# nilsfriess/dune-ddm

Measured on AMD Instinct MI355X. Metric: preconditioned CG iterations/sec (two-level additive Schwarz), 3D Poisson 10M DoF, higher is better.
Workload: dtype f64

## Files before the change

### dune-ddm_amd/__init__.py

```python
from __future__ import annotations

import ctypes
import os

import numpy as np

_HERE = os.path.dirname(os.path.abspath(__file__))
LIB_PATH = os.path.join(_HERE, "libddm_hip.so")

GENEO_AVAILABLE = True

DDM_OK, DDM_EINVAL, DDM_EHIP, DDM_ENOTIMPL, DDM_ENUMERIC, DDM_ECOMM = 0, -1, -2, -3, -4, -5
MULTI_ENGINES = ("levels", "xcd", "xcd1")


class DdmError(RuntimeError):
    def __init__(self, code, msg):
        super().__init__(f"ddm_hip error {code}: {msg}")
        self.code = code


class SolveResult(ctypes.Structure):
    _fields_ = [("iterations", ctypes.c_int32), ("converged", ctypes.c_int32), ("def0", ctypes.c_double),
                ("reduction", ctypes.c_double), ("elapsed_s", ctypes.c_double)]
# ... 43 lines not shown
    "ddm_galerkin_set_inverse": (_I32, [_P, _P, _P]),
    "ddm_csr_destroy": (None, [_P]),
    "ddm_csr_rows": (_I64, [_P]),
    "ddm_csr_nnz": (_I64, [_P]),
    "ddm_csr_mv": (_I32, [_P, _P, _P, _P]),
    "ddm_csr_usmv": (_I32, [_P, _P, _D, _P, _P]),
    "ddm_csr_mm": (_I32, [_P, _P, _I32, _P, _P]),
    "ddm_csr_row_order_tiled_host": (_I32, [_I64, _P, _P, _P, _P]),
    "ddm_dia_build_and_apply_host": (_I32, [_I64, _P, _P, _P, _P, _P, _I64, _P, _P]),
    "ddm_dia_windows_host": (_I32, [_I64, _P, _P, _P, _I64, _P, _I64, _P, _P]),
    "ddm_dia_codes_host": (_I32, [_I64, _P, _P, _P, _I32, _I64, _P, _P, _P, _P]),
    "ddm_ilu0_solve_multi": (_I32, [_P, _P, _I32, _P, _P]),
    "ddm_ilu0_solve_multi_f32": (_I32, [_P, _P, _I32, _P, _P]),
    "ddm_ilu0_create": (_I32, [_P, _P, _I64, _P, _PP]),
    "ddm_ilu0_destroy": (None, [_P]),
    "ddm_ilu0_solve": (_I32, [_P, _P, _P, _P]),
    "ddm_ilu0_debug_stamps": (_I32, [_P, _P, _P, _P, _P]),
    "ddm_ilu0_status": (_I32, [_P, _P, ctypes.POINTER(ctypes.c_int)]),
    "ddm_ilu0_peek_status": (_I32, [_P]),
    "ddm_ilu0_set_status": (_I32, [_P, _I32]),
    "ddm_halo_exchange_to": (_I32, [_P, _P, _P, _P]),
    "ddm_schwarz_local_solver": (_P, [_P]),
    "ddm_ilu0_pipe_trace": (_I32, [_P, _P, _P, _P, _P, _P, _I64, ctypes.POINTER(ctypes.c_int64)]),
    "ddm_ilu0_num_levels": (_I64, [_P, _I32]),
    "ddm_ilu0_wait": (_I32, [_P, _P]),
    "ddm_ilu0_box_check": (_I32, [_P, _P]),
    "ddm_ilu0_box_info": (_I32, [_P, _P, ctypes.c_int64, _P]),
    "ddm_ilu0_solve_tail": (_I32, [_P, _P, _P, _P, _P, _P]),
    "ddm_ilu0_engine": (_I32, [_P]),
    "ddm_chol_create": (_I32, [_P, _P, _I64, _P, _D, _PP]),
    "ddm_ilu0_is_direct": (_I32, [_P]),
    "ddm_ilu0_refinement": (_I32, [_P, _P]),
    "ddm_ilu0_sn_pivots": (_I32, [_P, _P, _P]),
    "ddm_sn_host_create": (_I32, [_I64, _P, _P, _I64, _P, _PP]),
    "ddm_sn_host_destroy": (None, [_P]),
    "ddm_sn_host_sizes": (_I32, [_P, _I64, _P, ctypes.POINTER(ctypes.c_double)]),
    "ddm_sn_host_get": (_I32, [_P, _I64, _P, _P, _P, _P, _P, _P]),
    "ddm_ilu0_nnz": (_I64, [_P]),
    "ddm_chol_host_create": (_I32, [_I64, _P, _P, _P, _I64, _P, _PP]),
    "ddm_direct_host_create": (_I32, [_I64, _P, _P, _P, _I64, _P, _I32, _PP]),
    "ddm_direct_create": (_I32, [_P, _P, _I64, _P, _I32, _D, _PP]),
    "ddm_chol_host_destroy": (None, [_P]),
    "ddm_chol_host_nnz": (_I64, [_P]),
    "ddm_chol_host_nnz_factor": (_I64, [_P]),
    "ddm_chol_host_flops": (_D, [_P]),
    "ddm_chol_host_get": (_I32, [_P, _P, _P, _P, _P]),
# ... 457 lines not shown
        return {"blocks": [tuple(int(v) for v in out[3 + 5 * b:8 + 5 * b]) for b in range(int(out[0]))], "grid": int(out[1]),
                "nested": SchwarzPreconditioner.ENGINES[int(out[2])] if out[2] >= 0 else None}

    def solve_tail(self, d, x, scale=None, add=None):
        self.ctx.check(self.ctx.lib.ddm_ilu0_solve_tail(self.ctx.h, self.h, _ptr(d), _ptr(x), _ptr(scale) if scale is not None else None,
                                                       _ptr(add) if add is not None else None))

    def wait(self):
        self.ctx.check(self.ctx.lib.ddm_ilu0_wait(self.ctx.h, self.h))

    def debug_stamps(self, d, x):
        out = np.zeros(8, dtype=np.uint64)
        self.ctx.check(self.ctx.lib.ddm_ilu0_debug_stamps(self.ctx.h, self.h, _ptr(d), _ptr(x), _hp(out)))
        return out

    def pipe_trace(self, d, x):
        nt = ctypes.c_int64()
        self.ctx.check(self.ctx.lib.ddm_ilu0_pipe_trace(self.ctx.h, self.h, None, None, None, None, 0, ctypes.byref(nt)))
        out = np.zeros((nt.value, 272), dtype=np.uint64)
        meta = np.zeros((nt.value, 2), dtype=np.int32)
        self.ctx.check(self.ctx.lib.ddm_ilu0_pipe_trace(self.ctx.h, self.h, _ptr(d), _ptr(x), _hp(out), _hp(meta), nt.value, ctypes.byref(nt)))
        return out, meta

    def engine(self):
        return SchwarzPreconditioner.ENGINES[int(self.ctx.lib.ddm_ilu0_engine(self.h))]

    def status(self):
        st = ctypes.c_int()
        self.ctx.check(self.ctx.lib.ddm_ilu0_status(self.ctx.h, self.h, ctypes.byref(st)))
        return st.value

    def factors(self):
        out = np.empty(self.nnz, dtype=np.float64)
        self.ctx.check(self.ctx.lib.ddm_ilu0_get_factors_host(self.ctx.h, self.h, _hp(out)))
        return out

    def __del__(self):
        try:
            if self.h and self.ctx.h:
                self.ctx.lib.ddm_ilu0_destroy(self.h)
        except Exception:
            pass


class Halo:
    COPY, ADD = 0, 1
# ... 756 lines not shown
```

### dune-ddm_amd/csrc/engine_pipe.hpp

```cpp

static int build_pipe_schedule(ddm_ctx *ctx, ddm_ilu0 *F)
{
  const ddm_csr *A = F->A;
  DDMCHECK(ilu0_sync_host_factor(ctx, F));
  pipe::Options opt;
  if (const char *e = std::getenv("DDM_PIPE_DELTA")) opt.delta = std::atoi(e);
  if (const char *e = std::getenv("DDM_PIPE_SPAN")) opt.max_span = std::atoi(e);
  if (const char *e = std::getenv("DDM_PIPE_REUSE")) opt.vote = std::atoi(e);
  int spread_env = -1;
  if (const char *e = std::getenv("DDM_PIPE_SPREAD")) spread_env = std::atoi(e);
  pipe::Schedule S;
  const int nb = (int)F->h_block_ptr.size() - 1;
  if (!pipe::build(A->nrows, A->h_rp.data(), A->h_ci.data(), F->h_lu.data(), F->h_diag.data(), nb, F->h_block_ptr.data(), opt, S)) {
    if (std::getenv("DDM_PIPE_VERBOSE")) std::fprintf(stderr, "[ddm] pipe engine not applicable: %s\n", S.error.c_str());
    return DDM_OK;
  }
  auto E = std::make_unique<PipeEngine>();
  E->ngroups = nb;
  E->stats = S.stats;
  E->spread = spread_env >= 0 ? spread_env : (nb < 8 && S.stats.max_rows_per_level > 48.0 * 64.0 ? 1 : 0);
  E->nposU = S.nposU;
  DDMCHECK(upload(ctx, S.groups.data(), (int64_t)S.groups.size(), E->groups));
  DDMCHECK(upload(ctx, S.tasks.data(), (int64_t)S.tasks.size(), E->tasks));
  DDMCHECK(upload(ctx, S.stream.data(), (int64_t)S.stream.size(), E->stream));
  DDMCHECK(upload(ctx, S.koff.data(), (int64_t)S.koff.size(), E->koff));
  DDMCHECK(upload(ctx, S.posU.data(), (int64_t)S.posU.size(), E->posU));
  {
    std::vector<int64_t> slot(S.slot[0]);
    slot.insert(slot.end(), S.slot[1].begin(), S.slot[1].end());
    DDMCHECK(upload(ctx, slot.data(), (int64_t)slot.size(), E->slot));
  }
  {
    std::vector<int32_t> rowU((size_t)std::max<int64_t>(S.nposU, 1), -1);
    for (size_t i = 0; i < S.posU.size(); ++i) rowU[(size_t)S.posU[i]] = (int32_t)i;
    DDMCHECK(upload(ctx, rowU.data(), (int64_t)rowU.size(), E->rowU));
  }
  HIPCHECK(ctx, E->ypos.alloc(S.nposL));
  HIPCHECK(ctx, E->xpos.alloc(S.nposU));
  HIPCHECK(ctx, dev_memset(E->ypos, 0, sizeof(double) * (size_t)std::max<int64_t>(S.nposL, 1)));
  HIPCHECK(ctx, dev_memset(E->xpos, 0, sizeof(double) * (size_t)std::max<int64_t>(S.nposU, 1)));
  const size_t pbytes = sizeof(unsigned long long) * 16 * std::max<size_t>(S.tasks.size(), 1);
  HIPCHECK(ctx, E->progress.alloc((int64_t)(pbytes / sizeof(unsigned long long))));
  HIPCHECK(ctx, dev_memset(E->progress, 0, pbytes));
  HIPCHECK(ctx, E->queue.alloc(32 * 4 * (int64_t)nb));
  HIPCHECK(ctx, dev_memset(E->queue, 0, sizeof(unsigned) * 32 * 4 * (size_t)nb));
  DDMCHECK(ilu0_alloc_xstate(ctx, F));
  HIPCHECK(ctx, hipFuncSetAttribute((const void *)k_trsv_pipe<false>, hipFuncAttributeMaxDynamicSharedMemorySize, (int)PIPE_LDS_BYTES));
  HIPCHECK(ctx, hipFuncSetAttribute((const void *)k_trsv_pipe<true>, hipFuncAttributeMaxDynamicSharedMemorySize, (int)PIPE_LDS_BYTES));
  int per_cu = 0;
  HIPCHECK(ctx, hipOccupancyMaxActiveBlocksPerMultiprocessor(&per_cu, (const void *)k_trsv_pipe<false>, 64 * PIPE_WAVES, PIPE_LDS_BYTES));
  per_cu = std::max(1, std::min(per_cu, 2));
  if (const char *e = std::getenv("DDM_PIPE_WG_PER_CU")) per_cu = std::max(1, std::min(per_cu, std::atoi(e)));
  E->grid = per_cu * (ctx->num_cu / 8 * 8);
  if (std::getenv("DDM_PIPE_VERBOSE")) {
    const pipe::Stats &st = S.stats;
    std::fprintf(stderr,
                 "[ddm] pipe schedule: %lld rows, tasks %lld+%lld, steps %lld+%lld (lane occupancy %.3f / %.3f), entries %lld: local %.3f self-global %.3f remote %.3f, "
                 "stream %.1f MB (%.2fx of 12 B/entry), max producers %lld, max steps %lld, regrouped %lld, levels <= %lld, rows/level <= %.0f, spread %d, grid %d\n",
                 (long long)st.rows, (long long)st.ntasks[0], (long long)st.ntasks[1], (long long)st.nsteps[0], (long long)st.nsteps[1],
                 (double)st.rows / (64.0 * std::max<int64_t>(st.nsteps[0], 1)), (double)st.rows / (64.0 * std::max<int64_t>(st.nsteps[1], 1)), (long long)st.entries,
                 (double)st.entries_local / std::max<int64_t>(st.entries, 1), (double)st.entries_self_global / std::max<int64_t>(st.entries, 1),
                 (double)st.entries_remote / std::max<int64_t>(st.entries, 1), S.stream.size() / 1e6, S.stream.size() / (12.0 * std::max<int64_t>(st.entries, 1)),
                 (long long)st.max_prod, (long long)st.max_steps, (long long)st.regrouped, (long long)st.max_levels, st.max_rows_per_level, E->spread, E->grid);
  }
  F->pipe = std::move(E);
  return DDM_OK;
}

static unsigned perm_grid(ddm_ctx *ctx, int64_t npos) { return (unsigned)std::max<int64_t>(1, std::min<int64_t>((npos + PERM_TILE - 1) / PERM_TILE, (int64_t)ctx->num_cu * 16)); }
static hipError_t enqueue_pipe(ddm_ctx *ctx, ddm_ilu0 *F, const double *d, double *x, unsigned *err, unsigned long long *stamps, const double *scale = nullptr,
                               const double *add = nullptr, hipEvent_t add_ready = nullptr)
{
  const PipeEngine &E = *F->pipe;
  PipeParams P;
  P.ngroups = E.ngroups;
  P.groups = E.groups;
  P.tasks = E.tasks;
  P.stream = E.stream;
  P.koff = E.koff;
  P.d = d;
  P.ypos = E.ypos;
  P.xpos = E.xpos;
  P.progress = E.progress;
  P.queue = E.queue;
  P.st = F->xstate;
  P.err = err;
// ... 11 lines not shown
```

### dune-ddm_amd/csrc/local_factor.hpp

```cpp

struct TriSchedule {
  int64_t nlev = 0;
  std::vector<LevelDesc> desc;
  dbuf<int32_t> rows;
  dbuf<int32_t> cols;
  dbuf<double> vals;
  dbuf<double> dinv;
  dbuf<float> vals_f32, dinv_f32;
  dbuf<LevelDesc> d_desc;
  struct Launch {
    int first, count;
    bool small;
  };
  std::vector<Launch> plan;
  int64_t ell_entries = 0;
  dbuf<int32_t> blk_off, blk_nlev;
  std::vector<int32_t> h_blk_nlev;
};

struct TriCsr {
  int64_t nlev = 0;
  std::vector<CsrLevel> desc;
  int64_t nrows = 0, entries = 0;
  dbuf<int32_t> rows;
// ... 33 lines not shown
  dbuf<GroupDesc> groups;
  dbuf<LevelDesc> desc;
  dbuf<int64_t> flag_off;
  dbuf<int32_t> rows, cols;
  dbuf<double> vals, dinv;
  dbuf<unsigned> flags;
  dbuf<double> dperm;
  dbuf<int64_t> lpos;
};

struct PipeEngine {
  int ngroups = 0;
  dbuf<pipe::Group> groups;
  dbuf<pipe::Task> tasks;
  dbuf<unsigned char> stream;
  dbuf<int32_t> koff, posU, rowU;
  dbuf<double> ypos, xpos;
  dbuf<unsigned long long> progress;
  dbuf<unsigned> queue;
  dbuf<int64_t> slot;
  int64_t nposU = 0;
  int spread = 0;
  int grid = 0;
  pipe::Stats stats;
};

struct BoxEngine {
  int nblocks = 0;
  int64_t nshell = 0, nprod = 0;
  dbuf<box::Block> blocks;
  dbuf<box::StepTab> steps;
  dbuf<double> stream;
  dbuf<unsigned long long> einfo;
  dbuf<double> E, ext_val;
  dbuf<int32_t> ext_col;
  dbuf<double> xs;
  dbuf<unsigned long long> prog;
  dbuf<unsigned> queue;
  unsigned long long *dbg = nullptr;
  int64_t n = 0, stream_len = 0, xs_len = 0, prog_len = 0, einfo_len = 0;
  dbuf<int64_t> srp;
  dbuf<int32_t> sci, srow;
  dbuf<double> sva, ds, xsol;
  ddm_csr *shell_csr = nullptr;
  ddm_ilu0 *shell = nullptr;
  int grid = 0;
// ... 147 lines not shown
```

### dune-ddm_amd/csrc/local_solve.hpp

```cpp

static int ilu0_prepare_engine(ddm_ctx *ctx, ddm_ilu0 *F)
{
  DDMCHECK(ilu0_join(ctx, F));
  if (F->engine == Engine::Box && F->box->shell) return ilu0_prepare_engine(ctx, F->box->shell);
  if (F->engine == Engine::Xcd2 && !F->xcd) return build_xcd_schedule(ctx, F);
  return DDM_OK;
}

static void enqueue_sn_panel(ddm_ctx *ctx, const ddm_ilu0 *F, int w, const double *D, int64_t ldd, double *X, int64_t ldx, double *work, double *yvec, unsigned *err)
{
  const SnDirect &S = *F->sn;
  const int64_t n = F->n;
  const dim3 grid(grid_for(n * w));
  hipLaunchKernelGGL(k_perm_gather, grid, dim3(WG), 0, ctx->stream, n, w, S.f->d_perm, D, ldd, work);
  sn::solve(*S.f, ctx->stream, w, work, w, yvec, err);
  hipLaunchKernelGGL(k_perm_scatter, grid, dim3(WG), 0, ctx->stream, n, w, S.f->d_perm, (const double *)work, X, ldx);
  for (int it = 0; it < S.refine_steps; ++it) {
    hipLaunchKernelGGL(k_residual_rowmajor, dim3((unsigned)((n * (int64_t)w + WG - 1) / WG)), dim3(WG), 0, ctx->stream, n, w, (const int64_t *)S.ref_rp, (const int32_t *)S.ref_ci,
                       (const double *)S.ref_va, (const double *)X, ldx, D, ldd, S.pr, (int64_t)w);
    hipLaunchKernelGGL(k_perm_gather, grid, dim3(WG), 0, ctx->stream, n, w, S.f->d_perm, (const double *)S.pr, (int64_t)w, work);
    sn::solve(*S.f, ctx->stream, w, work, w, yvec, err);
    hipLaunchKernelGGL(k_perm_scatter_add, grid, dim3(WG), 0, ctx->stream, n, w, S.f->d_perm, (const double *)work, X, ldx);
  }
}
// ... 74 lines not shown
  DDMCHECK(ilu0_join(ctx, F));
  if (!F->pipe) DDMCHECK(build_pipe_schedule(ctx, F));
  if (!F->pipe) return fail(ctx, DDM_EINVAL, "pipe engine not applicable to this matrix");
  const int64_t nt = F->pipe->stats.ntasks[0] + F->pipe->stats.ntasks[1];
  *ntasks = nt;
  if (!out_host) return DDM_OK;
  if (capacity_tasks < nt || !d || !x || d == x) return fail(ctx, DDM_EINVAL, "ddm_ilu0_pipe_trace: bad arguments");
  dbuf<unsigned long long> st;
  HIPCHECK(ctx, st.alloc(PIPE_STAMP_WORDS * (nt + 1)));
  HIPCHECK(ctx, hipMemsetAsync(st, 0, sizeof(unsigned long long) * PIPE_STAMP_WORDS * (size_t)(nt + 1), ctx->stream));
  (void)enqueue_pipe(ctx, F, d, x, F->err, st);
  int rc = ddm_memcpy_d2h(ctx, out_host, st, (int64_t)sizeof(unsigned long long) * PIPE_STAMP_WORDS * nt);
  if (!rc && meta_host) {
    std::vector<pipe::Task> tasks((size_t)nt);
    rc = ddm_memcpy_d2h(ctx, tasks.data(), F->pipe->tasks, (int64_t)sizeof(pipe::Task) * nt);
    for (int64_t t = 0; t < nt && !rc; ++t) {
      meta_host[2 * t] = tasks[(size_t)t].group;
      meta_host[2 * t + 1] = tasks[(size_t)t].sweep;
    }
  }
  return rc;
}

static int ilu0_is_pipe(ddm_ctx *ctx, ddm_ilu0 *F, bool *yes)
{
  *yes = false;
  if (!F || F->n == 0) return DDM_OK;
  DDMCHECK(ilu0_prepare_engine(ctx, F));
  *yes = F->engine == Engine::Pipe;
  return DDM_OK;
}

static int sn_check_valid(ddm_ctx *ctx, const ddm_ilu0 *F)
{
  if (F->sn && F->sn->invalid) return fail(ctx, DDM_ENUMERIC, "sparse direct solver (device): the factor is invalid after a failed refresh");
  return DDM_OK;
}

static int ilu0_solve_epilogue(ddm_ctx *ctx, ddm_ilu0 *F, const double *d, double *x, const double *scale, const double *add, hipEvent_t add_ready = nullptr)
{
  if (F && F->n == 0) return DDM_OK;
  if (!F || !d || !x || d == x) return fail(ctx, DDM_EINVAL, "ddm_ilu0_solve: bad arguments (d and x must not alias)");
  DDMCHECK(sn_check_valid(ctx, F));
  if (add_ready) {
    bool pipe_engine = false;
    DDMCHECK(ilu0_is_pipe(ctx, F, &pipe_engine));
// ... 97 lines not shown
```

### dune-ddm_amd/csrc/trsv_pipe_host.hpp

```cpp
#pragma once
#include "host_vec.hpp"
#include <algorithm>
#include <cstdint>
#include <cstring>
#include <functional>
#include <queue>
#include <string>
#include <thread>
#include <vector>

#if defined(__HIPCC__)
#define PIPE_HD __host__ __device__
#else
#define PIPE_HD
#endif

namespace pipe {

constexpr int LANES = 64;
constexpr int RING = 16;
constexpr int RING_Z = RING * LANES * 8;
constexpr int RING_BYTES = RING_Z + LANES * 8;
constexpr int ZERO_POS = RING_Z / 8;
constexpr int FIRST_POS = ZERO_POS + LANES;
constexpr int MIN_W = 14;
inline int32_t ring_op(int step, int lane) { return (int32_t)(((step % RING) * LANES + lane) * 8); }
constexpr int32_t PAD_OP = RING_Z;
constexpr int MAXPROD = 112;
constexpr int HDR_REQ0 = 8;
constexpr int MAX_W = 26;

struct Task {
  int64_t tile_off;
  int64_t pos_base;
  int64_t koff_base;
  int32_t nsteps, nprod, group, sweep;
  int32_t W, first_kib, pad0;
  int32_t start_level, pad[2];
  int32_t prod[MAXPROD];
};
static_assert(sizeof(Task) == 512, "Task layout");
struct Group {
  int32_t task0[2], ntask[2];
};

struct Geometry {
  int W = 0, idx_pieces = 0, val_pieces = 0, tile_bytes = 0;
  constexpr Geometry() = default;
  PIPE_HD constexpr explicit Geometry(int w_) : W(w_ > MIN_W ? w_ : MIN_W), idx_pieces((W + 3) / 4), val_pieces((W + 1) / 2), tile_bytes(1024 * (1 + idx_pieces + val_pieces)) {}
  static constexpr int FIXED_VAL = MIN_W / 2, FIXED_IDX = (MIN_W + 3) / 4, FIXED_KIB = 1 + FIXED_VAL + FIXED_IDX;
  PIPE_HD int val_piece(int q2) const { return q2 < FIXED_VAL ? 1 + q2 : FIXED_KIB + (q2 - FIXED_VAL); }
  PIPE_HD int idx_piece(int q4) const { return q4 < FIXED_IDX ? 1 + FIXED_VAL + q4 : FIXED_KIB + (val_pieces - FIXED_VAL) + (q4 - FIXED_IDX); }
  PIPE_HD int val_off(int u, int lane) const { return 1024 * val_piece(u >> 1) + lane * 16 + (u & 1) * 8; }
  PIPE_HD int idx_off(int u, int lane) const { return 1024 * idx_piece(u >> 2) + lane * 16 + (u & 3) * 4; }
};

PIPE_HD inline int64_t row_slot(int64_t tile_kib, int W, int lane) { return tile_kib << 16 | (int64_t)W << 8 | lane; }

struct Options {
  int delta = 24;
  int vote = 1;
  int pack_steps = 64;
  int max_span = 256;
};

struct Stats {
  int64_t ntasks[2] = {0, 0}, nsteps[2] = {0, 0};
  int64_t rows = 0, entries = 0, entries_local = 0, entries_self_global = 0, entries_remote = 0;
  int64_t max_prod = 0, max_steps = 0, regrouped = 0, nchains[2] = {0, 0};
  int64_t max_levels = 0;
  double max_rows_per_level = 0.0;
};

struct Schedule {
  Geometry geo;
  std::vector<Group> groups;
  std::vector<Task> tasks;
  hvec<unsigned char> stream;
  std::vector<int32_t> koff;
  std::vector<int32_t> rowL;
  std::vector<int32_t> posU;
  std::vector<int64_t> slot[2];
  int64_t nposL = 0, nposU = 0;
  Stats stats;
  std::string error;
};

namespace detail {

struct BlockSweep {
  struct TaskRec {
    int32_t start0 = 0, nsteps = 0, W = 1;
    std::vector<int32_t> stepW;
    std::vector<int32_t> rows;
    std::vector<int32_t> prod;
  };
  std::vector<TaskRec> tasks;
  std::vector<int32_t> task_of, step_of, lane_of;
  int64_t nchains = 0;
  bool cyclic = false, too_many_prod = false;
  int dissolve_rounds = 0;
  int32_t nlev = 0;
};

template <class Deps>
static void build_block_sweep(int64_t nb, bool upper, const Deps &deps, const Options &opt, BlockSweep &B)
{
  std::vector<int32_t> lev(nb, 0), chain(nb, -1), coff(nb, 0), ndep(nb, 0);
  std::vector<uint8_t> claimed(nb, 0), nochain(nb, 0);
  struct Chain {
    int32_t head, start, len;
  };
  std::vector<Chain> chains;
  std::vector<int64_t> cptr, pptr;
  std::vector<int32_t> crow(nb), pidx, freerows, comp;
  std::vector<uint8_t> is_free;
  int64_t nc = 0;
  int32_t ncomp = 0;
  auto sweep_key = [&](int32_t row) { return upper ? (int32_t)(nb - 1 - row) : row; };
  for (;;) {
    chains.clear();
    chains.reserve(nb / 16 + 16);
// ... 204 lines not shown
      return sweep_key(chains[a].head) < sweep_key(chains[b].head);
    });
    int32_t smin = 0x7fffffff, emax = 0;
    for (int64_t m = mptr[k]; m < mptr[k + 1]; ++m) {
      smin = std::min(smin, chains[members[m]].start);
      emax = std::max(emax, chains[members[m]].start + chains[members[m]].len);
    }
    bool fits = !protos.empty();
    if (fits) {
      const Proto &P = protos.back();
      if (std::max(P.end, emax) - std::min(P.start0, smin) > opt.max_span && !P.chains.empty()) fits = false;
      if (fits && opt.vote == 0 && (int)P.chains.size() + (int)(mptr[k + 1] - mptr[k]) > LANES) fits = false;
      if (fits) fits = place(mptr[k], mptr[k + 1], false);
    }
    if (!fits) new_task();
    place(mptr[k], mptr[k + 1], true);
    for (int64_t s = sptr[k]; s < sptr[k + 1]; ++s)
      if (--indeg[sidx[s]] == 0) ready.push(ckey[sidx[s]]);
  }
  if (emitted != ncomp) {
    B.cyclic = true;
    return;
  }
  const int64_t per_pack = (int64_t)opt.pack_steps * LANES;
  const int64_t npack = ((int64_t)freerows.size() + per_pack - 1) / per_pack;
  const int64_t ntask = npack + (int64_t)protos.size();
  B.task_of.assign(nb, -1);
  B.step_of.assign(nb, -1);
  B.lane_of.assign(nb, -1);
  for (int64_t f = 0; f < (int64_t)freerows.size(); ++f) {
    const int32_t i = freerows[f];
    B.task_of[i] = (int32_t)(f / per_pack);
    B.step_of[i] = (int32_t)((f % per_pack) / LANES);
    B.lane_of[i] = (int32_t)(f % LANES);
  }
  for (int64_t p = 0; p < (int64_t)protos.size(); ++p)
    for (size_t a = 0; a < protos[p].chains.size(); ++a) {
      const int32_t c = protos[p].chains[a];
      for (int32_t k = 0; k < chains[c].len; ++k) {
        const int32_t i = crow[cptr[c] + k];
        B.task_of[i] = (int32_t)(npack + p);
        B.step_of[i] = chains[c].start + k - protos[p].start0;
        B.lane_of[i] = protos[p].lanes[a];
      }
    }
  B.tasks.resize(ntask);
  for (int64_t t = 0; t < ntask; ++t) {
    auto &T = B.tasks[t];
    if (t < npack) {
      const int64_t cnt = std::min<int64_t>(per_pack, (int64_t)freerows.size() - t * per_pack);
      T.start0 = 0;
      T.nsteps = (int32_t)((cnt + LANES - 1) / LANES);
    } else {
      T.start0 = protos[t - npack].start0;
      T.nsteps = protos[t - npack].end - protos[t - npack].start0;
    }
    T.rows.assign((size_t)T.nsteps * LANES, -1);
    T.stepW.assign((size_t)T.nsteps, 1);
  }
  for (int64_t i = 0; i < nb; ++i) {
    const int32_t t = B.task_of[i];
    B.tasks[t].rows[(size_t)B.step_of[i] * LANES + B.lane_of[i]] = (int32_t)i;
    B.tasks[t].W = std::max(B.tasks[t].W, ndep[i]);
    B.tasks[t].stepW[B.step_of[i]] = std::max(B.tasks[t].stepW[B.step_of[i]], ndep[i]);
    deps(i, [&](int64_t j) {
      const int32_t tj = B.task_of[j];
      if (tj > t) B.cyclic = true;
      if (tj != t) B.tasks[t].prod.push_back(tj);
    });
  }
  for (auto &T : B.tasks) {
    std::sort(T.prod.begin(), T.prod.end());
    T.prod.erase(std::unique(T.prod.begin(), T.prod.end()), T.prod.end());
    if ((int)T.prod.size() > MAXPROD) B.too_many_prod = true;
  }
}

}

inline bool build(int64_t n, const int64_t *rp, const int32_t *ci, const double *lu, const int64_t *diag, int nblocks,
                  const int64_t *block_ptr, Options opt, Schedule &S, int nthreads = 0)
{
  using detail::BlockSweep;
  S = Schedule();
  int W = 1;
  for (int64_t i = 0; i < n; ++i) W = std::max<int>(W, (int)std::max(diag[i] - rp[i], rp[i + 1] - diag[i] - 1));
  if (W > MAX_W) {
    S.error = "triangular rows wider than the tile format";
    return false;
  }
// ... 26 lines not shown
      detail::build_block_sweep(nb, upper, deps, opt, B);
      Options o2 = opt;
      while (B.too_many_prod && !B.cyclic && o2.max_span > 24) {
        o2.max_span /= 2;
        B = BlockSweep();
        detail::build_block_sweep(nb, upper, deps, o2, B);
        regrouped[(size_t)b * 2 + sweep] += 1;
      }
    }
  });
  for (int b = 0; b < nblocks; ++b)
    for (int sweep = 0; sweep < 2; ++sweep) {
      const BlockSweep &B = BS[(size_t)b * 2 + sweep];
      if (B.cyclic) {
        S.error = "more than 64 mutually dependent chains";
        return false;
      }
      if (B.too_many_prod) {
        S.error = "a task has too many producer tasks";
        return false;
      }
      S.stats.regrouped += regrouped[(size_t)b * 2 + sweep];
      S.stats.nchains[sweep] += B.nchains;
      S.stats.max_levels = std::max<int64_t>(S.stats.max_levels, B.nlev);
      if (B.nlev > 0) S.stats.max_rows_per_level = std::max(S.stats.max_rows_per_level, (double)(block_ptr[b + 1] - block_ptr[b]) / B.nlev);
    }
  S.groups.resize(nblocks);
  std::vector<int64_t> task_base((size_t)nblocks * 2), pos_base((size_t)nblocks * 2);
  int64_t ntask = 0, npos[2] = {FIRST_POS, FIRST_POS}, nbytes = 0, nkoff = 0;
  for (int b = 0; b < nblocks; ++b)
    for (int sweep = 0; sweep < 2; ++sweep) {
      const BlockSweep &B = BS[(size_t)b * 2 + sweep];
      task_base[(size_t)b * 2 + sweep] = ntask;
      pos_base[(size_t)b * 2 + sweep] = npos[sweep];
      S.groups[b].task0[sweep] = (int32_t)ntask;
      S.groups[b].ntask[sweep] = (int32_t)B.tasks.size();
      ntask += (int64_t)B.tasks.size();
      for (const auto &T : B.tasks) {
        npos[sweep] += (int64_t)T.nsteps * LANES;
        for (int32_t w : T.stepW) nbytes += Geometry(w).tile_bytes;
        nkoff += T.nsteps + 1;
        S.stats.nsteps[sweep] += T.nsteps;
        S.stats.max_steps = std::max<int64_t>(S.stats.max_steps, T.nsteps);
        S.stats.max_prod = std::max<int64_t>(S.stats.max_prod, (int64_t)T.prod.size());
      }
      S.stats.ntasks[sweep] += (int64_t)B.tasks.size();
// ... 8 lines not shown
  }
  S.nposL = npos[0];
  S.nposU = npos[1];
  S.tasks.resize((size_t)ntask);
  S.stream.resize((size_t)nbytes);
  parallel_zero(S.stream.data(), (size_t)nbytes, (unsigned)nthreads);
  S.koff.assign((size_t)nkoff, 0);
  S.rowL.assign((size_t)npos[0], -1);
  S.posU.assign((size_t)n, 0);
  for (auto &sl : S.slot) sl.assign((size_t)n, 0);
  S.stats.rows = n;
  {
    int64_t off = 0, kb = 0;
    for (int b = 0; b < nblocks; ++b)
      for (int sweep = 0; sweep < 2; ++sweep) {
        const BlockSweep &B = BS[(size_t)b * 2 + sweep];
        int64_t pos = pos_base[(size_t)b * 2 + sweep];
        for (size_t q = 0; q < B.tasks.size(); ++q) {
          Task &T = S.tasks[(size_t)task_base[(size_t)b * 2 + sweep] + q];
          std::memset(&T, 0, sizeof(Task));
          T.tile_off = off;
          T.W = B.tasks[q].W;
          T.start_level = B.tasks[q].start0;
          T.koff_base = kb;
          int32_t k = 0;
          for (int32_t t = 0; t < B.tasks[q].nsteps; ++t) {
            S.koff[(size_t)kb + t] = k;
            k += Geometry(B.tasks[q].stepW[t]).tile_bytes / 1024;
          }
          S.koff[(size_t)kb + B.tasks[q].nsteps] = k;
          T.first_kib = S.koff[(size_t)kb + 1];
          kb += B.tasks[q].nsteps + 1;
          off += (int64_t)k * 1024;
          T.pos_base = pos;
          T.nsteps = B.tasks[q].nsteps;
          T.nprod = (int32_t)B.tasks[q].prod.size();
          T.group = b;
          T.sweep = sweep;
          for (int p = 0; p < T.nprod; ++p) T.prod[p] = (int32_t)(task_base[(size_t)b * 2 + sweep] + B.tasks[q].prod[p]);
          pos += (int64_t)T.nsteps * LANES;
        }
      }
  }
  std::vector<Stats> bstats((size_t)nblocks * 2);
  run_blocks([&](int b, int sweep) {
    const int64_t r0 = block_ptr[b];
// ... 72 lines not shown
  for (const Stats &b : bstats) {
    S.stats.entries += b.entries;
    S.stats.entries_local += b.entries_local;
    S.stats.entries_self_global += b.entries_self_global;
    S.stats.entries_remote += b.entries_remote;
  }
  return true;
}

inline void refresh_values(unsigned char *stream, const int64_t *slotL, const int64_t *slotU, int64_t n, const int64_t *rp, const int64_t *diag, const double *lu)
{
  for (int sweep = 0; sweep < 2; ++sweep)
    for (int64_t g = 0; g < n; ++g) {
      const int64_t word = (sweep ? slotU : slotL)[g];
      unsigned char *tile = stream + (word >> 16) * 1024;
      const Geometry G((int)(word >> 8 & 0xff));
      const int lane = (int)(word & 0xff);
      const int64_t k0 = sweep ? diag[g] + 1 : rp[g], k1 = sweep ? rp[g + 1] : diag[g];
      for (int64_t k = k0; k < k1; ++k) *reinterpret_cast<double *>(tile + G.val_off((int)(k - k0), lane)) = lu[k];
      if (sweep) *reinterpret_cast<double *>(tile + 512 + lane * 8) = lu[diag[g]];
    }
}

inline std::string emulate(const Schedule &S, int64_t n, const double *d, double *x)
{
  std::vector<double> ypos((size_t)S.nposL, 0.0), xpos((size_t)S.nposU, 0.0);
  std::vector<int32_t> done(S.tasks.size(), 0);
  std::vector<std::pair<int64_t, int32_t>> base[2];
  for (size_t t = 0; t < S.tasks.size(); ++t) base[S.tasks[t].sweep].push_back({S.tasks[t].pos_base, (int32_t)t});
  for (auto &b : base) std::sort(b.begin(), b.end());
  auto task_at = [&](int sweep, int64_t pos) {
    auto it = std::upper_bound(base[sweep].begin(), base[sweep].end(), std::make_pair(pos, (int32_t)0x7fffffff));
    return (it - 1)->second;
  };
  for (size_t g = 0; g < S.groups.size(); ++g)
    for (int sweep = 0; sweep < 2; ++sweep) {
      const bool upper = sweep == 1;
      const std::vector<double> &src = upper ? xpos : ypos;
      std::vector<double> &dst = upper ? xpos : ypos;
      for (int32_t q = 0; q < S.groups[g].ntask[sweep]; ++q) {
        const int32_t tid = S.groups[g].task0[sweep] + q;
        const Task &T = S.tasks[(size_t)tid];
        if (T.W > S.geo.W) return "tile geometry mismatch";
        std::vector<double> ring((size_t)RING_BYTES / 8, 0.0);
        std::vector<int32_t> prev_req(MAXPROD, 0);
        for (int p = 0; p < T.nprod; ++p)
          if (T.prod[p] >= tid || T.prod[p] < S.groups[g].task0[sweep]) return "producer is not earlier in the queue of its sweep";
        for (int32_t t = 0; t < T.nsteps; ++t) {
          const unsigned char *tile = S.stream.data() + T.tile_off + (int64_t)S.koff[(size_t)T.koff_base + t] * 1024;
          const int32_t *hdr = reinterpret_cast<const int32_t *>(tile);
          const Geometry G(hdr[2]);
          if (hdr[3] != (t + 1 < T.nsteps ? S.koff[(size_t)T.koff_base + t + 2] - S.koff[(size_t)T.koff_base + t + 1] : 0)) return "next-tile size mismatch";
          if (t == 0 && T.first_kib != S.koff[(size_t)T.koff_base + 1]) return "first-tile size mismatch";
          if (hdr[4] | hdr[5] | hdr[6] | hdr[7]) return "reserved header word is not zero";
          if (hdr[2] < MIN_W || G.W > std::max(T.W, MIN_W) || S.koff[(size_t)T.koff_base + t + 1] - S.koff[(size_t)T.koff_base + t] != G.tile_bytes / 1024) return "tile size mismatch";
          const int32_t *own = reinterpret_cast<const int32_t *>(tile + 256);
          const double *s0 = reinterpret_cast<const double *>(tile + 512);
          for (int p = 0; p < T.nprod; ++p) {
            const int32_t rq = (int32_t)(((uint32_t)hdr[HDR_REQ0 + p / 2] >> (16 * (p & 1))) & 0xffffu);
            if (rq < prev_req[p]) return "progress requirement decreases";
            if (rq > S.tasks[(size_t)T.prod[p]].nsteps) return "progress requirement beyond the producer's steps";
            prev_req[p] = rq;
          }
          double out[LANES];
          for (int l = 0; l < LANES; ++l) {
            const int64_t pos = T.pos_base + (int64_t)t * LANES + l;
            if (own[l] < 0 || own[l] % 8 || own[l] / 8 >= (upper ? S.nposL : n)) return "right-hand side operand out of range";
            if (!upper && S.rowL[(size_t)pos] >= 0 && own[l] / 8 != S.rowL[(size_t)pos]) return "right-hand side operand is not the row of the position";
            if (!upper && S.rowL[(size_t)pos] < 0 && own[l] != 0) return "padding lane with a right-hand side operand";
            double s = upper ? ypos[(size_t)own[l] / 8] : d[(size_t)own[l] / 8];
            for (int u = 0; u < G.W; ++u) {
              const int32_t op = *reinterpret_cast<const int32_t *>(tile + G.idx_off(u, l));
              const double a = *reinterpret_cast<const double *>(tile + G.val_off(u, l));
              double xv;
              if (op < 0 || op % 8) return "malformed operand";
              if (op <= RING_Z) {
                if (op < RING_Z) {
                  const int row = op / (LANES * 8);
                  int back = (t % RING) - row;
                  if (back <= 0) back += RING;
                  if (back > t) return "ring operand older than the task";
                }
                xv = ring[(size_t)op / 8];
              } else {
                const int64_t opos = op / 8;
                if (opos < FIRST_POS || opos >= (upper ? S.nposU : S.nposL)) return "position operand out of range";
                const int32_t pt = task_at(sweep, opos);
                const int32_t ps = (int32_t)((opos - S.tasks[(size_t)pt].pos_base) / LANES);
                if (pt == tid) {
                  if (ps >= t) return "own operand not yet computed";
                } else {
                  int p = 0;
                  while (p < T.nprod && T.prod[p] != pt) ++p;
                  if (p == T.nprod) return "operand of a task that is not a declared producer";
                  if (prev_req[p] < ps + 1) return "progress requirement does not cover an operand";
                  if (done[(size_t)pt] < ps + 1) return "producer has not run";
                }
                xv = src[(size_t)opos];
              }
              s -= a * xv;
            }
            out[l] = s * s0[l];
          }
          for (int l = 0; l < LANES; ++l) {
            ring[(size_t)(t % RING) * LANES + l] = out[l];
            dst[(size_t)(T.pos_base + (int64_t)t * LANES + l)] = out[l];
          }
          done[(size_t)tid] = t + 1;
        }
      }
    }
  for (int64_t i = 0; i < n; ++i) x[i] = xpos[(size_t)S.posU[(size_t)i]];
  return "";
}

}
```

### include/ddm_hip.h

```cpp
#ifndef DDM_HIP_H
#define DDM_HIP_H

#include <stdint.h>

#ifdef __cplusplus
extern "C" {
#endif

#define DDM_OK 0
#define DDM_EINVAL (-1)
#define DDM_EHIP (-2)
#define DDM_ENOTIMPL (-3)
#define DDM_ENUMERIC (-4)
#define DDM_ECOMM (-5)

typedef struct ddm_ctx ddm_ctx;
typedef struct ddm_csr ddm_csr;
typedef struct ddm_ilu0 ddm_ilu0;
typedef struct ddm_halo ddm_halo;
typedef struct ddm_op ddm_op;
typedef struct ddm_schwarz ddm_schwarz;
typedef struct ddm_galerkin ddm_galerkin;
typedef struct ddm_combined ddm_combined;

// ... 43 lines not shown
void ddm_ilu0_destroy(ddm_ilu0 *F);
int ddm_ilu0_refresh(ddm_ctx *ctx, ddm_ilu0 *F);
int ddm_ilu0_refresh_count(const ddm_ilu0 *F);
int ddm_ilu0_solve(ddm_ctx *ctx, ddm_ilu0 *F, const double *d, double *x);
int ddm_ilu0_solve_tail(ddm_ctx *ctx, ddm_ilu0 *F, const double *d, double *x, const double *scale, const double *add);
int ddm_ilu0_solve_multi(ddm_ctx *ctx, ddm_ilu0 *F, int nrhs, const double *D, double *X);
int ddm_ilu0_solve_multi_f32(ddm_ctx *ctx, ddm_ilu0 *F, int nrhs, const double *D, double *X);
int64_t ddm_ilu0_num_levels(const ddm_ilu0 *F, int upper);
int ddm_ilu0_status(ddm_ctx *ctx, const ddm_ilu0 *F, int *status);
int ddm_ilu0_peek_status(const ddm_ilu0 *F);
int ddm_ilu0_set_status(ddm_ilu0 *F, int status);
int ddm_ilu0_set_multi_engine(ddm_ctx *ctx, ddm_ilu0 *F, int mode);
int ddm_ilu0_multi_info(const ddm_ilu0 *F, int64_t *out, int64_t cap, int64_t *count);
int ddm_trsv_multi_plan_host(int64_t n, const int64_t *rp, const int32_t *ci, int64_t nblocks, const int64_t *block_ptr, int upper, int32_t *off, int64_t cap,
                             int32_t *blk_nlev, int64_t *nlev);
int ddm_trsv_multi_team_host(const uint32_t *tickets8, int nblocks, int force_one, int xcc, uint32_t xcd_ticket, uint32_t global_ticket, uint32_t grid, int32_t *out5);
int ddm_ilu0_engine(const ddm_ilu0 *F);
int ddm_ilu0_wait(ddm_ctx *ctx, ddm_ilu0 *F);
int ddm_ilu0_box_check(const ddm_ilu0 *F, unsigned long long *out1024);
int ddm_ilu0_box_info(const ddm_ilu0 *F, int64_t *out, int64_t capacity, int64_t *count);
int ddm_ilu0_debug_stamps(ddm_ctx *ctx, ddm_ilu0 *F, const double *d, double *x, unsigned long long *out6_host);
int ddm_ilu0_pipe_trace(ddm_ctx *ctx, ddm_ilu0 *F, const double *d, double *x, unsigned long long *out_host, int32_t *meta_host,
                        int64_t capacity_tasks, int64_t *ntasks);
int ddm_ilu0_get_factors_host(ddm_ctx *ctx, const ddm_ilu0 *F, double *lu_host);

int ddm_chol_create(ddm_ctx *ctx, const ddm_csr *A, int64_t nblocks, const int64_t *block_ptr, double max_flops, ddm_ilu0 **out);
int ddm_direct_create(ddm_ctx *ctx, const ddm_csr *A, int64_t nblocks, const int64_t *block_ptr, int general, double max_flops, ddm_ilu0 **out);
typedef struct ddm_sn_host ddm_sn_host;
int ddm_sn_host_create(int64_t n, const int64_t *rowptr, const int32_t *col, int64_t nblocks, const int64_t *block_ptr, ddm_sn_host **out);
void ddm_sn_host_destroy(ddm_sn_host *H);
int ddm_sn_host_sizes(const ddm_sn_host *H, int64_t block, int64_t *sizes, double *flops);
int ddm_sn_host_get(const ddm_sn_host *H, int64_t block, int32_t *perm, int32_t *first, int64_t *rptr, int32_t *rows, int32_t *parent, int32_t *level);
int ddm_ilu0_is_direct(const ddm_ilu0 *F);
int64_t ddm_ilu0_nnz(const ddm_ilu0 *F);
int ddm_ilu0_refinement(const ddm_ilu0 *F, double *omega);
int ddm_ilu0_sn_pivots(ddm_ctx *ctx, const ddm_ilu0 *F, int32_t *out_n);
typedef struct ddm_chol_host ddm_chol_host;
int ddm_chol_host_create(int64_t n, const int64_t *rowptr, const int32_t *col, const double *val, int64_t nblocks,
                         const int64_t *block_ptr, ddm_chol_host **out);
int ddm_direct_host_create(int64_t n, const int64_t *rowptr, const int32_t *col, const double *val, int64_t nblocks,
                           const int64_t *block_ptr, int general, ddm_chol_host **out);
void ddm_chol_host_destroy(ddm_chol_host *H);
int64_t ddm_chol_host_nnz(const ddm_chol_host *H);
int64_t ddm_chol_host_nnz_factor(const ddm_chol_host *H);
double ddm_chol_host_flops(const ddm_chol_host *H);
int ddm_chol_host_get(const ddm_chol_host *H, int32_t *perm, int64_t *rowptr, int32_t *col, double *lu);
// ... 219 lines not shown
```

Measured before the change: 242.8.

## Move late-starting pipe tasks earlier in the queue to cut dependency stalls

The pipelined triangular-solve scheduler now finds tasks whose start level sits far below the running maximum of earlier tasks and moves up to move_max of them forward in the per-block queue. The cap is derived from how many workgroups serve each queue. A moved task may depend on producers that come later in the queue, and this relies on enough concurrent workgroups holding tasks to avoid deadlock. The host emulator now simulates a limited number of slots to check for deadlock, and a pipe_info diagnostic exposes what was moved.

```diff
diff --git a/dune-ddm_amd/__init__.py b/dune-ddm_amd/__init__.py
--- a/dune-ddm_amd/__init__.py
+++ b/dune-ddm_amd/__init__.py
@@ -89,6 +89,7 @@
     "ddm_halo_exchange_to": (_I32, [_P, _P, _P, _P]),
     "ddm_schwarz_local_solver": (_P, [_P]),
     "ddm_ilu0_pipe_trace": (_I32, [_P, _P, _P, _P, _P, _P, _I64, ctypes.POINTER(ctypes.c_int64)]),
+    "ddm_ilu0_pipe_info": (_I32, [_P, _P, _P, _I64, ctypes.POINTER(ctypes.c_int64)]),
     "ddm_ilu0_num_levels": (_I64, [_P, _I32]),
     "ddm_ilu0_wait": (_I32, [_P, _P]),
     "ddm_ilu0_box_check": (_I32, [_P, _P]),
@@ -592,6 +593,16 @@
         self.ctx.check(self.ctx.lib.ddm_ilu0_pipe_trace(self.ctx.h, self.h, _ptr(d), _ptr(x), _hp(out), _hp(meta), nt.value, ctypes.byref(nt)))
         return out, meta
 
+    def pipe_info(self):
+        cnt = ctypes.c_int64()
+        self.ctx.check(self.ctx.lib.ddm_ilu0_pipe_info(self.ctx.h, self.h, None, 0, ctypes.byref(cnt)))
+        out = np.zeros(cnt.value, dtype=np.int64)
+        self.ctx.check(self.ctx.lib.ddm_ilu0_pipe_info(self.ctx.h, self.h, _hp(out), cnt.value, ctypes.byref(cnt)))
+        names = ("grid", "spread", "move_max", "moved_forward", "moved_backward", "max_moved", "move_gap", "ntasks")
+        info = dict(zip(names, out[:8].tolist()))
+        info["start_level"], info["moved"] = out[8::2].copy(), out[9::2].copy()
+        return info
+
     def engine(self):
         return SchwarzPreconditioner.ENGINES[int(self.ctx.lib.ddm_ilu0_engine(self.h))]
 
diff --git a/dune-ddm_amd/csrc/engine_pipe.hpp b/dune-ddm_amd/csrc/engine_pipe.hpp
--- a/dune-ddm_amd/csrc/engine_pipe.hpp
+++ b/dune-ddm_amd/csrc/engine_pipe.hpp
@@ -11,6 +11,20 @@
   if (const char *e = std::getenv("DDM_PIPE_SPREAD")) spread_env = std::atoi(e);
   pipe::Schedule S;
   const int nb = (int)F->h_block_ptr.size() - 1;
+  HIPCHECK(ctx, hipFuncSetAttribute((const void *)k_trsv_pipe<false>, hipFuncAttributeMaxDynamicSharedMemorySize, (int)PIPE_LDS_BYTES));
+  HIPCHECK(ctx, hipFuncSetAttribute((const void *)k_trsv_pipe<true>, hipFuncAttributeMaxDynamicSharedMemorySize, (int)PIPE_LDS_BYTES));
+  int per_cu = 0;
+  HIPCHECK(ctx, hipOccupancyMaxActiveBlocksPerMultiprocessor(&per_cu, (const void *)k_trsv_pipe<false>, 64 * PIPE_WAVES, PIPE_LDS_BYTES));
+  per_cu = std::max(1, std::min(per_cu, 2));
+  if (const char *e = std::getenv("DDM_PIPE_WG_PER_CU")) per_cu = std::max(1, std::min(per_cu, std::atoi(e)));
+  const int grid = per_cu * (ctx->num_cu / 8 * 8);
+  {
+    const int per_queue = std::min((grid / 8) / ((nb + 7) / 8), grid / std::max(nb, 1));
+    opt.move_max = std::min(per_queue / 2, 32);
+    if (per_queue - opt.move_max < 8) opt.move_max = 0;
+    if (const char *e = std::getenv("DDM_PIPE_MOVE")) opt.move_max = std::max(0, std::min(opt.move_max, std::atoi(e)));
+    if (const char *e = std::getenv("DDM_PIPE_MOVE_GAP")) opt.move_gap = std::atoi(e);
+  }
   if (!pipe::build(A->nrows, A->h_rp.data(), A->h_ci.data(), F->h_lu.data(), F->h_diag.data(), nb, F->h_block_ptr.data(), opt, S)) {
     if (std::getenv("DDM_PIPE_VERBOSE")) std::fprintf(stderr, "[ddm] pipe engine not applicable: %s\n", S.error.c_str());
     return DDM_OK;
@@ -45,23 +59,21 @@
   HIPCHECK(ctx, E->queue.alloc(32 * 4 * (int64_t)nb));
   HIPCHECK(ctx, dev_memset(E->queue, 0, sizeof(unsigned) * 32 * 4 * (size_t)nb));
   DDMCHECK(ilu0_alloc_xstate(ctx, F));
-  HIPCHECK(ctx, hipFuncSetAttribute((const void *)k_trsv_pipe<false>, hipFuncAttributeMaxDynamicSharedMemorySize, (int)PIPE_LDS_BYTES));
-  HIPCHECK(ctx, hipFuncSetAttribute((const void *)k_trsv_pipe<true>, hipFuncAttributeMaxDynamicSharedMemorySize, (int)PIPE_LDS_BYTES));
-  int per_cu = 0;
-  HIPCHECK(ctx, hipOccupancyMaxActiveBlocksPerMultiprocessor(&per_cu, (const void *)k_trsv_pipe<false>, 64 * PIPE_WAVES, PIPE_LDS_BYTES));
-  per_cu = std::max(1, std::min(per_cu, 2));
-  if (const char *e = std::getenv("DDM_PIPE_WG_PER_CU")) per_cu = std::max(1, std::min(per_cu, std::atoi(e)));
-  E->grid = per_cu * (ctx->num_cu / 8 * 8);
+  E->grid = grid;
+  E->move_max = opt.move_max;
+  E->move_gap = opt.move_gap;
   if (std::getenv("DDM_PIPE_VERBOSE")) {
     const pipe::Stats &st = S.stats;
     std::fprintf(stderr,
                  "[ddm] pipe schedule: %lld rows, tasks %lld+%lld, steps %lld+%lld (lane occupancy %.3f / %.3f), entries %lld: local %.3f self-global %.3f remote %.3f, "
-                 "stream %.1f MB (%.2fx of 12 B/entry), max producers %lld, max steps %lld, regrouped %lld, levels <= %lld, rows/level <= %.0f, spread %d, grid %d\n",
+                 "stream %.1f MB (%.2fx of 12 B/entry), max producers %lld, max steps %lld, regrouped %lld, levels <= %lld, rows/level <= %.0f, spread %d, grid %d, "
+                 "moved in the queues %lld+%lld (most in one %lld; at most %d, gap %d)\n",
                  (long long)st.rows, (long long)st.ntasks[0], (long long)st.ntasks[1], (long long)st.nsteps[0], (long long)st.nsteps[1],
                  (double)st.rows / (64.0 * std::max<int64_t>(st.nsteps[0], 1)), (double)st.rows / (64.0 * std::max<int64_t>(st.nsteps[1], 1)), (long long)st.entries,
                  (double)st.entries_local / std::max<int64_t>(st.entries, 1), (double)st.entries_self_global / std::max<int64_t>(st.entries, 1),
                  (double)st.entries_remote / std::max<int64_t>(st.entries, 1), S.stream.size() / 1e6, S.stream.size() / (12.0 * std::max<int64_t>(st.entries, 1)),
-                 (long long)st.max_prod, (long long)st.max_steps, (long long)st.regrouped, (long long)st.max_levels, st.max_rows_per_level, E->spread, E->grid);
+                 (long long)st.max_prod, (long long)st.max_steps, (long long)st.regrouped, (long long)st.max_levels, st.max_rows_per_level, E->spread, E->grid,
+                 (long long)st.moved[0], (long long)st.moved[1], (long long)st.max_moved, opt.move_max, opt.move_gap);
   }
   F->pipe = std::move(E);
   return DDM_OK;
diff --git a/dune-ddm_amd/csrc/local_factor.hpp b/dune-ddm_amd/csrc/local_factor.hpp
--- a/dune-ddm_amd/csrc/local_factor.hpp
+++ b/dune-ddm_amd/csrc/local_factor.hpp
@@ -79,6 +79,7 @@
   int64_t nposU = 0;
   int spread = 0;
   int grid = 0;
+  int move_max = 0, move_gap = 0;
   pipe::Stats stats;
 };
 
diff --git a/dune-ddm_amd/csrc/local_solve.hpp b/dune-ddm_amd/csrc/local_solve.hpp
--- a/dune-ddm_amd/csrc/local_solve.hpp
+++ b/dune-ddm_amd/csrc/local_solve.hpp
@@ -120,6 +120,28 @@
   return rc;
 }
 
+extern "C" int ddm_ilu0_pipe_info(ddm_ctx *ctx, ddm_ilu0 *F, int64_t *out, int64_t capacity, int64_t *count)
+{
+  if (!F || !count) return fail(ctx, DDM_EINVAL, "ddm_ilu0_pipe_info: bad arguments");
+  DDMCHECK(ilu0_join(ctx, F));
+  PipeEngine *E = F->pipe.get();
+  const int64_t nt = E ? E->stats.ntasks[0] + E->stats.ntasks[1] : 0;
+  *count = 8 + 2 * nt;
+  if (!out) return DDM_OK;
+  if (capacity < *count) return fail(ctx, DDM_EINVAL, "ddm_ilu0_pipe_info: capacity too small");
+  const int64_t v[8] = {E ? E->grid : 0, E ? E->spread : 0, E ? E->move_max : 0, E ? E->stats.moved[0] : 0, E ? E->stats.moved[1] : 0, E ? E->stats.max_moved : 0,
+                        E ? E->move_gap : 0, nt};
+  std::copy(v, v + 8, out);
+  if (!nt) return DDM_OK;
+  std::vector<pipe::Task> tasks((size_t)nt);
+  DDMCHECK(ddm_memcpy_d2h(ctx, tasks.data(), E->tasks, (int64_t)sizeof(pipe::Task) * nt));
+  for (int64_t t = 0; t < nt; ++t) {
+    out[8 + 2 * t] = tasks[(size_t)t].start_level;
+    out[9 + 2 * t] = tasks[(size_t)t].moved;
+  }
+  return DDM_OK;
+}
+
 static int ilu0_is_pipe(ddm_ctx *ctx, ddm_ilu0 *F, bool *yes)
 {
   *yes = false;
diff --git a/dune-ddm_amd/csrc/trsv_pipe_host.hpp b/dune-ddm_amd/csrc/trsv_pipe_host.hpp
--- a/dune-ddm_amd/csrc/trsv_pipe_host.hpp
+++ b/dune-ddm_amd/csrc/trsv_pipe_host.hpp
@@ -36,7 +36,7 @@
   int64_t koff_base;
   int32_t nsteps, nprod, group, sweep;
   int32_t W, first_kib, pad0;
-  int32_t start_level, pad[2];
+  int32_t start_level, moved, pad;
   int32_t prod[MAXPROD];
 };
 static_assert(sizeof(Task) == 512, "Task layout");
@@ -62,12 +62,16 @@
   int vote = 1;
   int pack_steps = 64;
   int max_span = 256;
+  int move_gap = 24;
+  int move_max = 32;
 };
 
 struct Stats {
   int64_t ntasks[2] = {0, 0}, nsteps[2] = {0, 0};
   int64_t rows = 0, entries = 0, entries_local = 0, entries_self_global = 0, entries_remote = 0;
   int64_t max_prod = 0, max_steps = 0, regrouped = 0, nchains[2] = {0, 0};
+  int64_t moved[2] = {0, 0};
+  int64_t max_moved = 0;
   int64_t max_levels = 0;
   double max_rows_per_level = 0.0;
 };
@@ -91,6 +95,7 @@
 struct BlockSweep {
   struct TaskRec {
     int32_t start0 = 0, nsteps = 0, W = 1;
+    bool moved = false;
     std::vector<int32_t> stepW;
     std::vector<int32_t> rows;
     std::vector<int32_t> prod;
@@ -98,6 +103,7 @@
   std::vector<TaskRec> tasks;
   std::vector<int32_t> task_of, step_of, lane_of;
   int64_t nchains = 0;
+  int32_t nmoved = 0;
   bool cyclic = false, too_many_prod = false;
   int dissolve_rounds = 0;
   int32_t nlev = 0;
@@ -348,6 +354,42 @@
     B.cyclic = true;
     return;
   }
+  std::vector<uint8_t> moved(protos.size(), 0);
+  if (opt.move_max > 0 && protos.size() > 1) {
+    std::vector<std::pair<int32_t, int32_t>> cand;
+    int32_t runmax = protos[0].start0;
+    for (int32_t p = 1; p < (int32_t)protos.size(); ++p) {
+      if (runmax - protos[p].start0 > opt.move_gap) cand.push_back({protos[p].start0 - runmax, p});
+      runmax = std::max(runmax, protos[p].start0);
+    }
+    std::sort(cand.begin(), cand.end());
+    if ((int)cand.size() > opt.move_max) cand.resize((size_t)opt.move_max);
+    if (!cand.empty()) {
+      for (auto &c : cand) {
+        moved[c.second] = 1;
+        c.first = protos[c.second].start0;
+      }
+      std::sort(cand.begin(), cand.end());
+      std::vector<int32_t> order;
+      order.reserve(protos.size());
+      size_t m = 0;
+      for (int32_t p = 0; p < (int32_t)protos.size(); ++p) {
+        if (moved[p]) continue;
+        while (m < cand.size() && cand[m].first < protos[p].start0) order.push_back(cand[m++].second);
+        order.push_back(p);
+      }
+      while (m < cand.size()) order.push_back(cand[m++].second);
+      std::vector<Proto> queued(protos.size());
+      std::vector<uint8_t> qmoved(protos.size());
+      for (size_t q = 0; q < order.size(); ++q) {
+        queued[q] = std::move(protos[order[q]]);
+        qmoved[q] = moved[order[q]];
+      }
+      protos.swap(queued);
+      moved.swap(qmoved);
+      B.nmoved = (int32_t)cand.size();
+    }
+  }
   const int64_t per_pack = (int64_t)opt.pack_steps * LANES;
   const int64_t npack = ((int64_t)freerows.size() + per_pack - 1) / per_pack;
   const int64_t ntask = npack + (int64_t)protos.size();
@@ -380,6 +422,7 @@
     } else {
       T.start0 = protos[t - npack].start0;
       T.nsteps = protos[t - npack].end - protos[t - npack].start0;
+      T.moved = moved[t - npack] != 0;
     }
     T.rows.assign((size_t)T.nsteps * LANES, -1);
     T.stepW.assign((size_t)T.nsteps, 1);
@@ -391,7 +434,7 @@
     B.tasks[t].stepW[B.step_of[i]] = std::max(B.tasks[t].stepW[B.step_of[i]], ndep[i]);
     deps(i, [&](int64_t j) {
       const int32_t tj = B.task_of[j];
-      if (tj > t) B.cyclic = true;
+      if (tj > t && !B.tasks[t].moved) B.cyclic = true;
       if (tj != t) B.tasks[t].prod.push_back(tj);
     });
   }
@@ -464,6 +507,8 @@
       }
       S.stats.regrouped += regrouped[(size_t)b * 2 + sweep];
       S.stats.nchains[sweep] += B.nchains;
+      S.stats.moved[sweep] += B.nmoved;
+      S.stats.max_moved = std::max<int64_t>(S.stats.max_moved, B.nmoved);
       S.stats.max_levels = std::max<int64_t>(S.stats.max_levels, B.nlev);
       if (B.nlev > 0) S.stats.max_rows_per_level = std::max(S.stats.max_rows_per_level, (double)(block_ptr[b + 1] - block_ptr[b]) / B.nlev);
     }
@@ -518,6 +563,7 @@
           T.tile_off = off;
           T.W = B.tasks[q].W;
           T.start_level = B.tasks[q].start0;
+          T.moved = B.tasks[q].moved ? 1 : 0;
           T.koff_base = kb;
           int32_t k = 0;
           for (int32_t t = 0; t < B.tasks[q].nsteps; ++t) {
@@ -636,7 +682,7 @@
     }
 }
 
-inline std::string emulate(const Schedule &S, int64_t n, const double *d, double *x)
+inline std::string emulate(const Schedule &S, int64_t n, const double *d, double *x, int slots = 0)
 {
   std::vector<double> ypos((size_t)S.nposL, 0.0), xpos((size_t)S.nposU, 0.0);
   std::vector<int32_t> done(S.tasks.size(), 0);
@@ -652,15 +698,47 @@
       const bool upper = sweep == 1;
       const std::vector<double> &src = upper ? xpos : ypos;
       std::vector<double> &dst = upper ? xpos : ypos;
-      for (int32_t q = 0; q < S.groups[g].ntask[sweep]; ++q) {
-        const int32_t tid = S.groups[g].task0[sweep] + q;
+      const int32_t task0 = S.groups[g].task0[sweep], ntask = S.groups[g].ntask[sweep];
+      struct Held {
+        int32_t tid = -1, t = 0;
+        std::vector<double> ring;
+        std::vector<int32_t> prev_req;
+      };
+      int nslots = slots;
+      if (nslots <= 0) {
+        nslots = 1;
+        for (int32_t q = 0; q < ntask; ++q) nslots += S.tasks[(size_t)(task0 + q)].moved ? 1 : 0;
+      }
+      std::vector<Held> held((size_t)std::min<int64_t>(nslots, ntask));
+      int32_t next = 0, finished = 0;
+      auto dequeue = [&](Held &H) -> std::string {
+        H.tid = -1;
+        while (next < ntask && H.tid < 0) {
+          const int32_t tid = task0 + next++;
+          const Task &T = S.tasks[(size_t)tid];
+          if (T.W > S.geo.W) return "tile geometry mismatch";
+          for (int p = 0; p < T.nprod; ++p) {
+            if (T.prod[p] == tid || T.prod[p] < task0 || T.prod[p] >= task0 + ntask) return "producer is not another task of the queue of its sweep";
+            if (T.prod[p] > tid && !T.moved) return "producer is not earlier in the queue of its sweep";
+          }
+          if (T.nsteps <= 0) {
+            ++finished;
+            continue;
+          }
+          H.tid = tid;
+          H.t = 0;
+          H.ring.assign((size_t)RING_BYTES / 8, 0.0);
+          H.prev_req.assign(MAXPROD, 0);
+        }
+        return "";
+      };
+      auto advance = [&](Held &H, bool &ran) -> std::string {
+        const int32_t tid = H.tid, t = H.t;
         const Task &T = S.tasks[(size_t)tid];
-        if (T.W > S.geo.W) return "tile geometry mismatch";
-        std::vector<double> ring((size_t)RING_BYTES / 8, 0.0);
-        std::vector<int32_t> prev_req(MAXPROD, 0);
-        for (int p = 0; p < T.nprod; ++p)
-          if (T.prod[p] >= tid || T.prod[p] < S.groups[g].task0[sweep]) return "producer is not earlier in the queue of its sweep";
-        for (int32_t t = 0; t < T.nsteps; ++t) {
+        std::vector<double> &ring = H.ring;
+        std::vector<int32_t> &prev_req = H.prev_req;
+        ran = false;
+        {
           const unsigned char *tile = S.stream.data() + T.tile_off + (int64_t)S.koff[(size_t)T.koff_base + t] * 1024;
           const int32_t *hdr = reinterpret_cast<const int32_t *>(tile);
           const Geometry G(hdr[2]);
@@ -674,8 +752,11 @@
             const int32_t rq = (int32_t)(((uint32_t)hdr[HDR_REQ0 + p / 2] >> (16 * (p & 1))) & 0xffffu);
             if (rq < prev_req[p]) return "progress requirement decreases";
             if (rq > S.tasks[(size_t)T.prod[p]].nsteps) return "progress requirement beyond the producer's steps";
-            prev_req[p] = rq;
-          }
+          }
+          for (int p = 0; p < T.nprod; ++p)
+            if ((int32_t)(((uint32_t)hdr[HDR_REQ0 + p / 2] >> (16 * (p & 1))) & 0xffffu) > done[(size_t)T.prod[p]]) return "";
+          for (int p = 0; p < T.nprod; ++p) prev_req[p] = (int32_t)(((uint32_t)hdr[HDR_REQ0 + p / 2] >> (16 * (p & 1))) & 0xffffu);
+          ran = true;
           double out[LANES];
           for (int l = 0; l < LANES; ++l) {
             const int64_t pos = T.pos_base + (int64_t)t * LANES + l;
@@ -722,6 +803,29 @@
           }
           done[(size_t)tid] = t + 1;
         }
+        H.t = t + 1;
+        return "";
+      };
+      for (Held &H : held) {
+        const std::string e = dequeue(H);
+        if (!e.empty()) return e;
+      }
+      while (finished < ntask) {
+        bool any = false;
+        for (Held &H : held) {
+          if (H.tid < 0) continue;
+          bool ran = false;
+          std::string e = advance(H, ran);
+          if (!e.empty()) return e;
+          if (!ran) continue;
+          any = true;
+          if (H.t == S.tasks[(size_t)H.tid].nsteps) {
+            ++finished;
+            e = dequeue(H);
+            if (!e.empty()) return e;
+          }
+        }
+        if (!any && finished < ntask) return "queue order deadlocks with " + std::to_string(nslots) + " slots";
       }
     }
   for (int64_t i = 0; i < n; ++i) x[i] = xpos[(size_t)S.posU[(size_t)i]];
diff --git a/include/ddm_hip.h b/include/ddm_hip.h
--- a/include/ddm_hip.h
+++ b/include/ddm_hip.h
@@ -89,6 +89,7 @@
 int ddm_ilu0_debug_stamps(ddm_ctx *ctx, ddm_ilu0 *F, const double *d, double *x, unsigned long long *out6_host);
 int ddm_ilu0_pipe_trace(ddm_ctx *ctx, ddm_ilu0 *F, const double *d, double *x, unsigned long long *out_host, int32_t *meta_host,
                         int64_t capacity_tasks, int64_t *ntasks);
+int ddm_ilu0_pipe_info(ddm_ctx *ctx, ddm_ilu0 *F, int64_t *out, int64_t capacity, int64_t *count);
 int ddm_ilu0_get_factors_host(ddm_ctx *ctx, const ddm_ilu0 *F, double *lu_host);
 
 int ddm_chol_create(ddm_ctx *ctx, const ddm_csr *A, int64_t nblocks, const int64_t *block_ptr, double max_flops, ddm_ilu0 **out);
```

Measured after the change: 259.1, median of 6. 6.7% higher.
